# hguo/ftk

Hardware: AMD Instinct MI355X
Metric: space-time simplices/sec (higher is better)
Workload: dtype int64

## Files before the change

ftk_amd/__init__.py:

```python
import ctypes as C

import numpy as np

from . import _lib
from ._lib import (CP_DTYPE, FORMAT_BINARY, FORMAT_JSON, FORMAT_TEXT, SCOPE_BOTH, SCOPE_INTERVAL, SCOPE_ORDINAL, SOURCE_DERIVED, SOURCE_GIVEN, SOURCE_NONE,
                   TAG_EXACT64, TAG_REFERENCE, TAG_WORK_INDEX, FtkxError, Options, Stats)

__all__ = ["trace_curves", "pass2", "trace_and_post_process", "post_process", "post_process_curves", "TrajectorySet", "write_critical_points", "read_critical_points",
           "write_traced_critical_points", "read_traced_critical_points", "Context", "CriticalPointTracker2DRegular", "CriticalPointTracker3DRegular", "extract_cp2dt", "extract_cp3dt",
           "scaling_factor", "gaussian_kernel", "gaussian_kernel1d", "CP_DTYPE", "FtkxError"]


def _ptr(a):
    if a is None:
        return None, None, 0, False
    if isinstance(a, int):
        return a, None, 1, False
    if hasattr(a, "data_ptr"):
        if a.dtype.is_floating_point and a.element_size() not in (4, 8):
            raise TypeError("fields must be float64 or float32")
        a = a.contiguous()
        return a.data_ptr(), a, 1 if a.is_cuda else 0, bool(a.dtype.is_floating_point and a.element_size() == 4)
    if isinstance(a, np.ndarray) and a.dtype == np.float32:
        a = np.ascontiguousarray(a)
# ... 471 lines not shown

    def sweep_collect(self, copy=True):
        out, n = C.c_void_p(), C.c_size_t()
        self._ck(self._L.ftkx_sweep_collect(self._h, C.byref(out), C.byref(n)))
        return _lib.records_from(out.value, n.value, copy)

    def stats(self):
        s = Stats()
        self._ck(self._L.ftkx_get_stats(self._h, C.byref(s)))
        return {k: getattr(s, k) for k, _ in Stats._fields_}

    KERNELS = ("mask_kernel", "cull_kernel", "exact_kernel", "tile_kernel")

    def invalidate_masks(self):
        self._ck(self._L.ftkx_invalidate_masks(self._h))

    def set_profiling(self, on=True):
        self._ck(self._L.ftkx_set_profiling(self._h, int(on)))

    def debug_tile_repeat(self, repeat):
        self._ck(self._L.ftkx_debug_tile_repeat(self._h, int(repeat)))

    def upload_counts(self):
        a = C.c_ulonglong(0); b = C.c_ulonglong(0)
        self._ck(self._L.ftkx_debug_upload_counts(self._h, C.byref(a), C.byref(b)))
        return int(a.value), int(b.value)

    def kernel_times(self):
        ms = (C.c_double * 4)(); n = (C.c_ulonglong * 4)()
        self._ck(self._L.ftkx_get_kernel_times(self._h, ms, n))
# ... 571 lines not shown
```

ftk_amd/_lib.py:

```python
import ctypes as C
import os

import numpy as np

_HERE = os.path.dirname(os.path.abspath(__file__))
LIB_PATH = os.path.join(_HERE, "libftkx.so")

CP_DTYPE = np.dtype([("x", "<f8", (3,)), ("t", "<f8"), ("scalar", "<f8", (3,)), ("type", "<u4"), ("aux", "<u4"), ("tag", "<u8")])
assert CP_DTYPE.itemsize == 72

OK, E_INVALID, E_DEVICE, E_NOMEM, E_NOSLICE, E_UNSUPPORTED = 0, -1, -2, -3, -4, -5
SCOPE_ORDINAL, SCOPE_INTERVAL, SCOPE_BOTH = 1, 2, 3
TAG_WORK_INDEX, TAG_REFERENCE, TAG_EXACT64 = 0, 1, 2
FORMAT_BINARY, FORMAT_JSON, FORMAT_TEXT = 0, 1, 2
SOURCE_NONE, SOURCE_GIVEN, SOURCE_DERIVED = 0, 1, 2


class Options(C.Structure):
    _fields_ = [("jacobian_symmetric", C.c_int), ("robust", C.c_int), ("use_type_filter", C.c_int), ("type_filter", C.c_uint),
                ("compute_degrees", C.c_int), ("tag_mode", C.c_int), ("exact_only", C.c_int), ("derive_jacobian", C.c_int),
                ("coords_mode", C.c_int), ("coords_bounds", C.c_double * 6)]


class Stats(C.Structure):
# ... 44 lines not shown
    _fields_ = [("rank", C.c_int), ("nranks", C.c_int), ("t0", C.c_int), ("t1", C.c_int), ("lower", C.c_int), ("upper", C.c_int), ("bytes_sent", C.c_ulonglong),
                ("bytes_received", C.c_ulonglong), ("fallbacks", C.c_int), ("last_asked", C.c_longlong), ("last_served", C.c_longlong), ("last_path", C.c_int),
                ("last_status", C.c_ulonglong), ("open", C.c_int)]


class FtkxError(RuntimeError):
    def __init__(self, code, msg):
        super().__init__(f"ftkx error {code}: {msg}")
        self.code = code


EXPORTS = [
    "ftkx_create", "ftkx_destroy", "ftkx_last_error", "ftkx_set_stream", "ftkx_set_options", "ftkx_default_options", "ftkx_set_mesh",
    "ftkx_push_slice", "ftkx_push_scalar_slice", "ftkx_drop_slice", "ftkx_slice_resolution", "ftkx_slices_resolution", "ftkx_slices_prepare", "ftkx_sweep_announce", "ftkx_set_slice_resolution", "ftkx_export_masks_size", "ftkx_export_masks", "ftkx_push_masked_slice", "ftkx_packed_masks_bytes", "ftkx_export_masks_packed", "ftkx_push_masked_slice_packed", "ftkx_sweep_cull", "ftkx_get_sparse_cells", "ftkx_patch_doubles", "ftkx_gather_patches", "ftkx_scatter_patches", "ftkx_scaling_factor",
    "ftkx_sweep", "ftkx_sweep_series", "ftkx_sweep_series_submit", "ftkx_sweep_series_complete", "ftkx_sweep_series_abort", "ftkx_series_dist_cells", "ftkx_series_dist_begin", "ftkx_series_dist_cull", "ftkx_series_dist_serve", "ftkx_series_dist_finish", "ftkx_series_dist_status", "ftkx_series_last_path", "ftkx_series_split_decision", "ftkx_sweep_enqueue", "ftkx_sweep_enqueue_many", "ftkx_sweep_collect", "ftkx_sweep_cancel", "ftkx_get_stats", "ftkx_invalidate_masks", "ftkx_debug_stream_read", "ftkx_debug_tile_repeat", "ftkx_set_profiling", "ftkx_get_kernel_times", "ftkx_extract_cp2dt", "ftkx_extract_cp3dt", "ftkx_free",
    "ftkx_trace_curves", "ftkx_trace_curves_ctx", "ftkx_trace_curves_tags_ctx", "ftkx_trace_curves_device", "ftkx_trace_last_path", "ftkx_free_curves", "ftkx_post_process_curves", "ftkx_post_process_curves_device", "ftkx_pass2_device", "ftkx_post_process_last_path", "ftkx_free_trajectories", "ftkx_format_from_path", "ftkx_write_critical_points", "ftkx_read_critical_points", "ftkx_write_traced_critical_points", "ftkx_read_traced_critical_points", "ftkx_gradient2D", "ftkx_jacobian2D", "ftkx_gradient3D", "ftkx_jacobian3D", "ftkx_gaussian_kernel", "ftkx_conv2D", "ftkx_conv3D", "ftkx_set_spatial_smoothing", "ftkx_tracker_set_spatial_smoothing", "ftkx_debug_conv_relaunch", "ftkx_gaussian_kernel1d", "ftkx_temporal_combine", "ftkx_set_temporal_smoothing", "ftkx_temporal_push", "ftkx_temporal_flush", "ftkx_debug_temporal_relaunch", "ftkx_tracker_set_temporal_smoothing", "ftkx_tracker_snapshots_from_last_push", "ftkx_tracker_flush_temporal_smoothing", "ftkx_tracker_reset", "ftkx_version", "ftkx_device_count", "ftkx_pointer_device", "ftkx_context_device", "ftkx_last_mask_kernel", "ftkx_debug_mask_kernel_launches", "ftkx_debug_upload_counts", "ftkx_debug_mask_relaunch",
    "ftkx_push_scalar_slice_f32", "ftkx_push_slice_f32", "ftkx_temporal_push_f32", "ftkx_widen_f32", "ftkx_conv2D_f32", "ftkx_conv3D_f32", "ftkx_debug_widen_relaunch", "ftkx_debug_f32_counts", "ftkx_debug_array_counts",
    "ftkx_push_slice_planar", "ftkx_push_slice_planar_f32", "ftkx_temporal_push_planar", "ftkx_temporal_push_planar_f32", "ftkx_concat", "ftkx_concat_f32", "ftkx_debug_concat_relaunch", "ftkx_debug_planar_counts",
    "ftkx_tracker_push_vector_field_components", "ftkx_tracker_push_vector_field_components_f32",
    "ftkx_debug_series_order", "ftkx_debug_sort_records",
    "ftkx_set_perturbation", "ftkx_set_clamp", "ftkx_adjust", "ftkx_adjust_f32", "ftkx_debug_adjust_relaunch", "ftkx_debug_adjust_counts", "ftkx_tracker_set_perturbation", "ftkx_tracker_set_clamp",
    "ftkx_push_aux_slice", "ftkx_push_aux_slice_f32", "ftkx_sample_aux", "ftkx_debug_sample_relaunch", "ftkx_debug_sample_counts",
    "ftkx_tracker_set_scalar_components", "ftkx_tracker_push_snapshot_extra", "ftkx_tracker_get_curve_scalars",
    "ftkx_tracker_push_scalar_field_snapshot_f32", "ftkx_tracker_push_vector_field_snapshot_f32", "ftkx_tracker_push_field_data_snapshot_f32",
    "ftkx_tracker_post_process", "ftkx_tracker_get_curve_points", "ftkx_tracker_write", "ftkx_tracker_read_critical_points",
    "ftkx_tracker_create", "ftkx_tracker_create_multi", "ftkx_tracker_sync", "ftkx_tracker_destroy", "ftkx_tracker_last_error", "ftkx_tracker_set_domain", "ftkx_tracker_set_array_domain",
    "ftkx_tracker_set_sources", "ftkx_tracker_set_flags", "ftkx_tracker_set_stream", "ftkx_tracker_set_current_timestep", "ftkx_tracker_set_enable_streaming_trajectories", "ftkx_tracker_set_deferred_collection", "ftkx_tracker_set_trace_on_device", "ftkx_tracker_trace_last_path", "ftkx_tracker_set_post_process_on_device", "ftkx_tracker_post_process_last_path", "ftkx_tracker_set_communicator", "ftkx_tracker_set_slab_transport", "ftkx_tracker_set_slab_hub", "ftkx_online_tracer_create", "ftkx_online_tracer_destroy", "ftkx_online_tracer_grow", "ftkx_online_tracer_curves", "ftkx_tracker_set_coords_bounds", "ftkx_tracker_set_coords_rectilinear", "ftkx_tracker_set_coords_explicit", "ftkx_set_coords_rectilinear", "ftkx_set_coords_explicit", "ftkx_tracker_initialize",
    "ftkx_tracker_push_scalar_field_snapshot", "ftkx_tracker_push_vector_field_snapshot", "ftkx_tracker_push_field_data_snapshot",
    "ftkx_tracker_advance_timestep", "ftkx_tracker_update_timestep", "ftkx_tracker_num_critical_points",
    "ftkx_tracker_get_critical_points", "ftkx_tracker_get_scaling", "ftkx_tracker_get_stats",
    "ftkx_tracker_finalize", "ftkx_tracker_num_curves", "ftkx_tracker_get_curves",
# ... 28 lines not shown
    L.ftkx_push_scalar_slice.argtypes = [vp, C.c_int, dbl, C.c_int]
    L.ftkx_drop_slice.argtypes = [vp, C.c_int]
    L.ftkx_slice_resolution.argtypes = [vp, C.c_int, C.POINTER(C.c_double), C.POINTER(C.c_double)]
    L.ftkx_set_slice_resolution.argtypes = [vp, C.c_int, C.c_double, C.c_double]
    L.ftkx_scaling_factor.argtypes = [C.c_double, C.POINTER(C.c_int)]; L.ftkx_scaling_factor.restype = C.c_ulonglong
    L.ftkx_sweep.argtypes = [vp, C.c_int, C.c_int, C.c_ulonglong, C.POINTER(vp), C.POINTER(C.c_size_t)]
    L.ftkx_sweep_enqueue.argtypes = [vp, C.c_int, C.c_int, C.c_ulonglong]
    L.ftkx_sweep_collect.argtypes = [vp, C.POINTER(vp), C.POINTER(C.c_size_t)]
    L.ftkx_get_stats.argtypes = [vp, C.POINTER(Stats)]
    L.ftkx_set_profiling.argtypes = [vp, C.c_int]
    L.ftkx_invalidate_masks.argtypes = [vp]
    L.ftkx_debug_stream_read.argtypes = [vp, vp, C.c_size_t]
    L.ftkx_debug_tile_repeat.argtypes = [vp, C.c_int]
    L.ftkx_debug_upload_counts.argtypes = [vp, C.POINTER(C.c_ulonglong), C.POINTER(C.c_ulonglong)]
    L.ftkx_debug_mask_relaunch.argtypes = [vp, C.c_int, C.c_int, C.c_int, C.c_int, C.POINTER(C.c_double)]
    L.ftkx_series_split_decision.argtypes = [vp, C.POINTER(C.c_int), C.POINTER(C.c_double), C.POINTER(C.c_double)]
    L.ftkx_get_kernel_times.argtypes = [vp, C.POINTER(C.c_double), C.POINTER(C.c_ulonglong)]
    L.ftkx_extract_cp2dt.argtypes = [C.c_int, C.c_int] + [ll3] * 6 + [dbl] * 6 + [C.c_int, dbl, C.c_ulonglong, C.POINTER(Options), C.c_int, C.POINTER(vp), C.POINTER(C.c_size_t)]
    L.ftkx_extract_cp3dt.argtypes = [C.c_int, C.c_int] + [ll3] * 6 + [dbl] * 6 + [C.c_ulonglong, C.POINTER(Options), C.c_int, C.POINTER(vp), C.POINTER(C.c_size_t)]
    L.ftkx_free.argtypes = [vp]; L.ftkx_free.restype = None
    L.ftkx_trace_curves.argtypes = [C.c_int, ll3, ll3, vp, C.c_size_t, C.POINTER(Curves)]
    L.ftkx_trace_curves_ctx.argtypes = [vp, C.c_int, ll3, ll3, vp, C.c_size_t, C.POINTER(Curves)]
    L.ftkx_trace_curves_tags_ctx.argtypes = [vp, C.c_int, ll3, ll3, vp, C.c_size_t, C.POINTER(Curves)]
    L.ftkx_trace_curves_device.argtypes = [vp, C.c_int, ll3, ll3, vp, C.c_size_t, C.c_int, C.POINTER(Curves)]
    L.ftkx_trace_last_path.argtypes = [vp]
    L.ftkx_free_curves.argtypes = [C.POINTER(Curves)]; L.ftkx_free_curves.restype = None
    L.ftkx_post_process_curves.argtypes = [vp, C.c_size_t, C.POINTER(Curves), C.POINTER(Trajectories)]
    L.ftkx_post_process_curves_device.argtypes = [vp, vp, C.c_size_t, C.POINTER(Curves), C.POINTER(Trajectories)]
    L.ftkx_pass2_device.argtypes = [vp, C.c_int, ll3, ll3, vp, C.c_size_t, C.POINTER(Curves), C.POINTER(Trajectories)]
    L.ftkx_post_process_last_path.argtypes = [vp]
# ... 196 lines not shown
```

ftk_amd/csrc/mask_kernels.hip:

```cpp
#include <atomic>
#include "internal.hpp"
#include "mask_plan.hpp"
#include "sweep_device.hpp"
#include "series_device.hpp"

namespace ftkx {

__device__ inline void red_commit(u64 *red, double mn, double mx, unsigned slot)
{
  for (int o = 32; o > 0; o >>= 1) { mn = fmin(mn, __shfl_down(mn, o)); mx = fmax(mx, __shfl_down(mx, o)); }
  if ((threadIdx.x & 63) == 0) {
    atomicMin(&red[2 * (slot & 63u)], (u64)__double_as_longlong(mn));
    atomicMax(&red[2 * (slot & 63u) + 1], (u64)__double_as_longlong(mx));
  }
}

template <int ND>
__global__ __launch_bounds__(kThreads) void mask_kernel(const Mesh m, const MaskJob *__restrict__ jobs)
{
  const MaskJob job = jobs[blockIdx.y];
  const int P = m.mask_pitch, DH = m.ext_sz[1], DD = (ND == 3) ? m.ext_sz[2] : 1;
  const size_t n = (size_t)P * DH * DD;
  double red_mn = DBL_MAX, red_mx = 0.0;
  for (size_t idx = (size_t)blockIdx.x * kThreads + threadIdx.x; idx < n; idx += (size_t)gridDim.x * kThreads) {
    const int i = (int)(idx % P), j = (int)((idx / P) % DH), k = (int)(idx / ((size_t)P * DH));
    unsigned char mk = kNeutral;
    if (i < m.ext_sz[0]) {
      const int vx[3] = {i + m.ext_st[0], j + m.ext_st[1], k + m.ext_st[2]};
      bool in_dom = true;
      for (int d = 0; d < ND; d ++) in_dom = in_dom && vx[d] >= m.dom_lb[d] && vx[d] <= m.dom_ub[d];
      double v[ND];
      vector_at<ND>(m, job.S, job.V, i, j, k, v);
      unsigned bits = 0;
// ... 97 lines not shown
#define FTKX_GLOBAL __attribute__((address_space(1)))

__device__ inline double dpp_lower_or(double v, double edge)
{
  const long long b = __double_as_longlong(v), e = __double_as_longlong(edge);
  const int lo = __builtin_amdgcn_update_dpp((int)e, (int)b, 0x138 , 0xf, 0xf, false);
  const int hi = __builtin_amdgcn_update_dpp((int)(e >> 32), (int)(b >> 32), 0x138, 0xf, 0xf, false);
  return __longlong_as_double(((long long)hi << 32) | (unsigned)lo);
}
__device__ inline double dpp_upper_or(double v, double edge)
{
  const long long b = __double_as_longlong(v), e = __double_as_longlong(edge);
  const int lo = __builtin_amdgcn_update_dpp((int)e, (int)b, 0x130 , 0xf, 0xf, false);
  const int hi = __builtin_amdgcn_update_dpp((int)(e >> 32), (int)(b >> 32), 0x130, 0xf, 0xf, false);
  return __longlong_as_double(((long long)hi << 32) | (unsigned)lo);
}

__device__ inline void remap_block(int swizzle, unsigned &bx, unsigned &by, unsigned &bz)
{
  bx = blockIdx.x; by = blockIdx.y; bz = blockIdx.z;
  if (swizzle & 1) {
    const unsigned nb = gridDim.x * gridDim.y * gridDim.z;
    unsigned b = blockIdx.x + gridDim.x * (blockIdx.y + gridDim.y * blockIdx.z);
    const unsigned per = nb / 8, rem = nb % 8, xcd = b % 8, k = b / 8;
    b = xcd * per + (xcd < rem ? xcd : rem) + k;
    bx = b % gridDim.x; by = (b / gridDim.x) % gridDim.y; bz = b / (gridDim.x * gridDim.y);
  }
  if (swizzle & 8) {
    const unsigned YG = ((unsigned)swizzle >> 8) & 0xffu;
    const unsigned nb = gridDim.x * gridDim.y * gridDim.z, G = gridDim.x * YG;
// ... 80 lines not shown
  return __longlong_as_double(((long long)hi << 32) | (unsigned)lo);
}

__device__ inline unsigned word_summary(unsigned bits)
{
  unsigned q;
  asm("v_and_b32_sdwa %0, %1, %1 dst_sel:DWORD dst_unused:UNUSED_PAD src0_sel:BYTE_0 src1_sel:BYTE_1\n\t"
      "s_nop 1\n\t"
      "v_and_b32_dpp %0, %0, %0 quad_perm:[1,0,3,2] row_mask:0xf bank_mask:0xf\n\t"
      "s_nop 1\n\t"
      "v_and_b32_dpp %0, %0, %0 quad_perm:[2,3,0,1] row_mask:0xf bank_mask:0xf"
      : "=&v"(q) : "v"(bits));
  return q;
}

__device__ inline double max_abs2(double a, double b) { double r; asm("v_max_f64 %0, |%1|, |%2|" : "=v"(r) : "v"(a), "v"(b)); return r; }
__device__ inline double max_with_abs(double acc, double b) { asm("v_max_f64 %0, %0, |%1|" : "+v"(acc) : "v"(b)); return acc; }
__device__ inline double max_plain(double acc, double b) { asm("v_max_f64 %0, %0, %1" : "+v"(acc) : "v"(b)); return acc; }

template <int ND>
__device__ inline unsigned guard_and_reduce(unsigned a0, unsigned a1, double dx0, double dx1, double dy0, double dy1, double dz0, double dz1,
                                            bool rv, unsigned cmask, bool per_vertex_rule, double tbig, double h, double &acc0, double &acc1, double &red_mn)
{
  double m0 = max_abs2(dx0, dy0), m1 = max_abs2(dx1, dy1);
  if constexpr (ND == 3) { m0 = max_with_abs(m0, dz0); m1 = max_with_abs(m1, dz1); }
  unsigned bits = a0 | (a1 << 8);
  if (rv) {
    acc0 = max_plain(acc0, m0); acc1 = max_plain(acc1, m1);
    const unsigned u = bits | (bits >> 3);
    if (__builtin_amdgcn_ballot_w64((~u & cmask) != 0u)) {
      auto take = [&](double d) { const double a = fabs(h * d); red_mn = fmin(red_mn, a == 0.0 ? DBL_MAX : a); };
      if (cmask & 0x00ffu) { take(dx0); take(dy0); if (ND == 3) take(dz0); }
      if (cmask & 0xff00u) { take(dx1); take(dy1); if (ND == 3) take(dz1); }
// ... 958 lines not shown
  case MASK_ROWS2: hipLaunchKernelGGL(mask_rows2_kernel<8>, grid, block, 0, stream, m, d_jobs, p.groups, p.swizzle); break;
  case MASK_REDUCE:
    if (m.nd == 2) hipLaunchKernelGGL((mask_march4_kernel<2, true, 1, 8>), grid, block, 0, stream, m, d_jobs, p.zchunk, p.swizzle);
    else hipLaunchKernelGGL((mask_march4_kernel<3, true, 1, 4>), grid, block, 0, stream, m, d_jobs, p.zchunk, p.swizzle);
    break;
  case MASK_MARCH4: hipLaunchKernelGGL((mask_march4_kernel<2, false, 1, 8>), grid, block, 0, stream, m, d_jobs, p.zchunk, p.swizzle); break;
  case MASK_VEC2:
    if (m.nd == 2) hipLaunchKernelGGL(mask_vec2_kernel<2>, grid, block, 0, stream, m, d_jobs);
    else hipLaunchKernelGGL(mask_vec2_kernel<3>, grid, block, 0, stream, m, d_jobs);
    break;
  case MASK_VEC:
    if (m.nd == 2) hipLaunchKernelGGL(mask_vec_kernel<2>, grid, block, 0, stream, m, d_jobs);
    else hipLaunchKernelGGL(mask_vec_kernel<3>, grid, block, 0, stream, m, d_jobs);
    break;
  default:
    if (m.nd == 2) hipLaunchKernelGGL(mask_kernel<2>, grid, block, 0, stream, m, d_jobs);
    else hipLaunchKernelGGL(mask_kernel<3>, grid, block, 0, stream, m, d_jobs);
  }
}

void launch_masks(const Mesh &m, const MaskJob *d_jobs, int njobs, hipStream_t stream) { launch_masks_impl(m, d_jobs, njobs, false, stream); }
void launch_reduce_march(const Mesh &m, const MaskJob *d_jobs, int njobs, hipStream_t stream) { launch_masks_impl(m, d_jobs, njobs, true, stream); }

}
```

ftk_amd/csrc/mask_plan.hpp:

```cpp
#pragma once
#include <algorithm>
#include <cstdlib>
#include <cstring>
#include <vector>

namespace ftkx {

struct ZPlan {
  unsigned npieces;
  unsigned z0[47], len[47];
  unsigned sgroup;
};

#if defined(__HIPCC__)
#define FTKX_PLAN_HD __host__ __device__
#else
#define FTKX_PLAN_HD
#endif

struct ZWhere { unsigned job, piece; };
FTKX_PLAN_HD inline ZWhere zplan_decode(const ZPlan &plan, int njobs, unsigned bz)
{
  ZWhere w;
  if (njobs >= 0) { w.piece = bz / (unsigned)njobs; w.job = bz - w.piece * (unsigned)njobs; return w; }
  const unsigned nj = (unsigned)-njobs, t = bz / plan.npieces;
  if (plan.sgroup == 0) { w.piece = bz - t * plan.npieces; w.job = t; return w; }
  const unsigned ngroups = (nj + plan.sgroup - 1) / plan.sgroup, small = nj / ngroups, extra = nj - small * ngroups, head = extra * (small + 1);
  const unsigned size = t < head ? small + 1 : small;
  const unsigned first = t < head ? t / size * size : head + (t - head) / size * size;
  const unsigned r = bz - first * plan.npieces;
  w.piece = r / size; w.job = first + (r - w.piece * size);
  return w;
}

constexpr long kHookUnset = -0x7fffffffL;
struct MaskHooks {
  long swizzle = kHookUnset, yg = kHookUnset, zchunk = kHookUnset, lmin = kHookUnset, lcap = kHookUnset, order = kHookUnset, sgroup = kHookUnset, rows = kHookUnset, lean = kHookUnset;
  long u_rows = 0;
};
inline long hook_or(long v, long dflt) { return v == kHookUnset ? dflt : v; }

inline MaskHooks parse_mask_hooks(const char *plan, const char *u_rows)
{
  MaskHooks h;
  const struct { const char *name; long MaskHooks::*knob; } knobs[] = {{"swizzle", &MaskHooks::swizzle}, {"yg", &MaskHooks::yg}, {"zchunk", &MaskHooks::zchunk},
    {"lmin", &MaskHooks::lmin}, {"lcap", &MaskHooks::lcap}, {"order", &MaskHooks::order}, {"sgroup", &MaskHooks::sgroup}, {"rows", &MaskHooks::rows}, {"lean", &MaskHooks::lean}};
  for (const char *p = plan ? plan : ""; *p;) {
    while (*p == ',' || *p == ' ') p ++;
    for (const auto &k : knobs) {
      const size_t n = strlen(k.name);
      if (!strncmp(p, k.name, n) && p[n] == '=' && h.*k.knob == kHookUnset) h.*k.knob = atol(p + n + 1);
    }
    while (*p && *p != ',') p ++;
  }
  if (u_rows) h.u_rows = atoi(u_rows);
  return h;
}
inline MaskHooks read_mask_hooks() { return parse_mask_hooks(getenv("FTKX_MASK_PLAN"), getenv("FTKX_U_ROWS")); }

struct MaskShape { int nd, scalar_mode, ext_sz[3], mask_pitch; };

enum MaskFamily { MASK_MARCH6 = 0 , MASK_MARCH4 = 1 , MASK_ROWS2 = 2 ,
                  MASK_REDUCE = 3 , MASK_VEC2 = 4 ,
                  MASK_VEC = 5 , MASK_GENERIC = 6, MASK_FAMILIES = 7 };
constexpr unsigned kMaskThreads = 256;

struct MaskPlan {
  MaskFamily family;
  const char *name;
  bool march2;
  bool has_summary;
  int u_rows;
  unsigned grid[3], block, lds_bytes;
  int swizzle, zchunk, groups, njobs;
  ZPlan z;
};

inline MaskPlan plan_masks(const MaskShape &s, const MaskHooks &h, int njobs, bool reduce)
{
  MaskPlan p = MaskPlan();
  const int DW = s.ext_sz[0], DH = s.ext_sz[1], DD = s.nd == 3 ? s.ext_sz[2] : 1;
  const size_t nrows = (size_t)DH * (size_t)DD;
  p.march2 = s.scalar_mode && (DW % 2) == 0 && DW >= 2 && (size_t)DW * nrows * 8 < (1ull << 32);
  const bool vec_fast = !s.scalar_mode && DW >= 8 && (DW % 8) == 0;
  const bool vec_lean = vec_fast && DW >= 256 && hook_or(h.lean, 1) != 0 && (size_t)DW * nrows * 8 * (size_t)s.nd < (1ull << 31) && (size_t)s.mask_pitch * nrows < (1ull << 31);
  p.has_summary = h.u_rows >= 0 && (s.scalar_mode ? p.march2 && (DW % 8) == 0 : vec_fast);
  if (!p.has_summary || h.u_rows == 1) p.u_rows = 1;
  else if (!s.scalar_mode) p.u_rows = vec_lean ? 4 : 1;
  else if (s.nd == 3) p.u_rows = h.u_rows == 4 ? 4 : 16;
  else p.u_rows = 4;
// ... 81 lines not shown
  if (vec_fast) {
    const size_t groups = (size_t)(DW / 4) * nrows;
    size_t bx = (groups + kMaskThreads - 1) / kMaskThreads;
    if (bx > 2048) bx = 2048;
    while (bx > 256 && bx * kMaskThreads * 4 > groups) bx /= 2;
    if (p.u_rows == 4) {
      const size_t units = (size_t)((DW / 4 + 63) / 64) * ((DH + 3) / 4) * (size_t)DD;
      bx = (units + 7) / 8;
      if (bx > 2048) bx = 2048;
    }
    p.grid[0] = (unsigned)bx;
    p.family = p.u_rows == 4 ? MASK_VEC2 : MASK_VEC;
    p.name = p.u_rows == 4 ? (s.nd == 2 ? "ftkx::mask_vec2_kernel<2>" : "ftkx::mask_vec2_kernel<3>") : (s.nd == 2 ? "ftkx::mask_vec_kernel<2>" : "ftkx::mask_vec_kernel<3>");
    return p;
  }
  const size_t n = (size_t)s.mask_pitch * nrows;
  size_t bx = (n + kMaskThreads - 1) / kMaskThreads;
  if (bx > 4096) bx = 4096;
  p.grid[0] = (unsigned)bx;
  p.family = MASK_GENERIC; p.name = s.nd == 2 ? "ftkx::mask_kernel<2>" : "ftkx::mask_kernel<3>";
  return p;
}

}
```

ftk_amd/csrc/prepare.hip:

```cpp
#include "ctx.hpp"

using namespace ftkxh;

namespace ftkxh {

__global__ void init_red_kernel(u64 *red, size_t nslots, u64 *counters)
{
  const size_t i = (size_t)blockIdx.x * blockDim.x + threadIdx.x;
  if (i < nslots) { red[2 * i] = 0x7fefffffffffffffull; red[2 * i + 1] = 0ull; }
  if (counters && i < (size_t)ftkx::CNT_N) counters[i] = 0ull;
}

__global__ __launch_bounds__(256) void readback_kernel(const u64 *__restrict__ red, u64 *dst, unsigned k, unsigned *flag, unsigned seq)
{
  const unsigned wv = threadIdx.x >> 6, lane = threadIdx.x & 63;
  for (unsigned base = wv * 8; base < k; base += 32) {
    u64 mn[8], mx[8];
#pragma unroll
    for (int j = 0; j < 8; j ++) {
      const unsigned i = base + j < k ? base + j : k - 1;
      mn[j] = red[(size_t)i * 128 + 2 * lane]; mx[j] = red[(size_t)i * 128 + 2 * lane + 1];
    }
#pragma unroll
    for (int j = 0; j < 8; j ++) {
// ... 201 lines not shown
    hipStream_t q = st[r % nstreams];
    if (with_begin) launch_fetch_desc(c->h_desc.p, (char *)c->d_desc.p + 4096, 4096, q);
    ftkx::launch_masks(m, (const MaskJob *)c->d_desc.p, 1, q);
  }
  if (nstreams == 2) { HIP_TRY(c, hipEventRecord(eb, st[1])); HIP_TRY(c, hipStreamWaitEvent(st[0], eb, 0)); }
  HIP_TRY(c, hipEventRecord(e1, st[0]));
  HIP_TRY(c, hipEventSynchronize(e1));
  float ms = 0.f;
  HIP_TRY(c, hipEventElapsedTime(&ms, e0, e1));
  (void)hipEventDestroy(e0); (void)hipEventDestroy(e1); (void)hipEventDestroy(eb);
  if (st[1]) aux_stream_put(c, false, st[1]);
  *ms_per_launch = (double)ms / reps;
  return FTKX_OK;
}

int ftkx_sweep_announce(ftkx_ctx *c, const int *ts, const int *scopes, int n)
{
  if (!c || (n > 0 && (!ts || !scopes))) return fail(c, FTKX_E_INVALID, "null argument");
  c->announced.clear();
  for (int i = 0; i < n; i ++) {
    if (scopes[i] < FTKX_SCOPE_ORDINAL || scopes[i] > FTKX_SCOPE_BOTH) { c->announced.clear(); return fail(c, FTKX_E_INVALID, "ftkx_sweep_announce: bad scope %d", scopes[i]); }
    c->announced.push_back({ts[i], scopes[i]});
  }
  return FTKX_OK;
}

}
```

include/ftkx.h:

```cpp
#ifndef FTKX_H
#define FTKX_H

#include <stddef.h>

#ifdef __cplusplus
extern "C" {
#endif

typedef struct ftkx_cp_t {
  double x[3];
  double t;
  double scalar[3];
  unsigned int type;
  unsigned long long tag;
} ftkx_cp_t;

static inline unsigned int ftkx_cp_aux(const ftkx_cp_t *cp) { return ((const unsigned int *)cp)[15]; }
static inline int ftkx_cp_ordinal(const ftkx_cp_t *cp) { return (int)(ftkx_cp_aux(cp) & 1u); }
static inline int ftkx_cp_timestep(const ftkx_cp_t *cp) { return (int)(ftkx_cp_aux(cp) >> 1); }

typedef struct ftkx_ctx ftkx_ctx;

enum {
  FTKX_OK = 0,
// ... 215 lines not shown
int ftkx_debug_series_order(const ftkx_ctx *ctx, unsigned long long out[4]);
int ftkx_debug_sort_records(ftkx_ctx *ctx, const ftkx_cp_t *in, size_t n, int key_bits, ftkx_cp_t *out);

int ftkx_debug_stream_read(ftkx_ctx *ctx, const void *device_ptr, size_t bytes);

int ftkx_debug_tile_repeat(ftkx_ctx *ctx, int repeat);

const char *ftkx_last_mask_kernel(void);

int ftkx_debug_mask_kernel_launches(unsigned long long *launches, const char **names, int n);

int ftkx_debug_upload_counts(const ftkx_ctx *ctx, unsigned long long *staged, unsigned long long *direct);

int ftkx_debug_mask_relaunch(ftkx_ctx *ctx, int t, int reps, int nstreams, int with_begin, double *ms_per_launch);

const char *ftkx_version(void);
int ftkx_device_count(void);
int ftkx_pointer_device(const void *p);
int ftkx_context_device(const ftkx_ctx *ctx);

#ifdef __cplusplus
}
#endif
#endif
```

Measured before the change: 45990 billion.

## Replace generic byte mask kernel with wave-strided row-run tiled mask kernel

```diff
diff --git a/ftk_amd/__init__.py b/ftk_amd/__init__.py
--- a/ftk_amd/__init__.py
+++ b/ftk_amd/__init__.py
@@ -509,6 +509,10 @@
 
     def invalidate_masks(self):
         self._ck(self._L.ftkx_invalidate_masks(self._h))
+
+    def debug_mask_slices(self, ts, threshold, big, M_ptr, red_ptr):
+        ts = [int(t) for t in ts]
+        self._ck(self._L.ftkx_debug_mask_slices(self._h, (C.c_int * len(ts))(*ts), len(ts), float(threshold), float(big), M_ptr, red_ptr))
 
     def set_profiling(self, on=True):
         self._ck(self._L.ftkx_set_profiling(self._h, int(on)))
diff --git a/ftk_amd/_lib.py b/ftk_amd/_lib.py
--- a/ftk_amd/_lib.py
+++ b/ftk_amd/_lib.py
@@ -82,7 +82,7 @@
     "ftkx_create", "ftkx_destroy", "ftkx_last_error", "ftkx_set_stream", "ftkx_set_options", "ftkx_default_options", "ftkx_set_mesh",
     "ftkx_push_slice", "ftkx_push_scalar_slice", "ftkx_drop_slice", "ftkx_slice_resolution", "ftkx_slices_resolution", "ftkx_slices_prepare", "ftkx_sweep_announce", "ftkx_set_slice_resolution", "ftkx_export_masks_size", "ftkx_export_masks", "ftkx_push_masked_slice", "ftkx_packed_masks_bytes", "ftkx_export_masks_packed", "ftkx_push_masked_slice_packed", "ftkx_sweep_cull", "ftkx_get_sparse_cells", "ftkx_patch_doubles", "ftkx_gather_patches", "ftkx_scatter_patches", "ftkx_scaling_factor",
     "ftkx_sweep", "ftkx_sweep_series", "ftkx_sweep_series_submit", "ftkx_sweep_series_complete", "ftkx_sweep_series_abort", "ftkx_series_dist_cells", "ftkx_series_dist_begin", "ftkx_series_dist_cull", "ftkx_series_dist_serve", "ftkx_series_dist_finish", "ftkx_series_dist_status", "ftkx_series_last_path", "ftkx_series_split_decision", "ftkx_sweep_enqueue", "ftkx_sweep_enqueue_many", "ftkx_sweep_collect", "ftkx_sweep_cancel", "ftkx_get_stats", "ftkx_invalidate_masks", "ftkx_debug_stream_read", "ftkx_debug_tile_repeat", "ftkx_set_profiling", "ftkx_get_kernel_times", "ftkx_extract_cp2dt", "ftkx_extract_cp3dt", "ftkx_free",
-    "ftkx_trace_curves", "ftkx_trace_curves_ctx", "ftkx_trace_curves_tags_ctx", "ftkx_trace_curves_device", "ftkx_trace_last_path", "ftkx_free_curves", "ftkx_post_process_curves", "ftkx_post_process_curves_device", "ftkx_pass2_device", "ftkx_post_process_last_path", "ftkx_free_trajectories", "ftkx_format_from_path", "ftkx_write_critical_points", "ftkx_read_critical_points", "ftkx_write_traced_critical_points", "ftkx_read_traced_critical_points", "ftkx_gradient2D", "ftkx_jacobian2D", "ftkx_gradient3D", "ftkx_jacobian3D", "ftkx_gaussian_kernel", "ftkx_conv2D", "ftkx_conv3D", "ftkx_set_spatial_smoothing", "ftkx_tracker_set_spatial_smoothing", "ftkx_debug_conv_relaunch", "ftkx_gaussian_kernel1d", "ftkx_temporal_combine", "ftkx_set_temporal_smoothing", "ftkx_temporal_push", "ftkx_temporal_flush", "ftkx_debug_temporal_relaunch", "ftkx_tracker_set_temporal_smoothing", "ftkx_tracker_snapshots_from_last_push", "ftkx_tracker_flush_temporal_smoothing", "ftkx_tracker_reset", "ftkx_version", "ftkx_device_count", "ftkx_pointer_device", "ftkx_context_device", "ftkx_last_mask_kernel", "ftkx_debug_mask_kernel_launches", "ftkx_debug_upload_counts", "ftkx_debug_mask_relaunch",
+    "ftkx_trace_curves", "ftkx_trace_curves_ctx", "ftkx_trace_curves_tags_ctx", "ftkx_trace_curves_device", "ftkx_trace_last_path", "ftkx_free_curves", "ftkx_post_process_curves", "ftkx_post_process_curves_device", "ftkx_pass2_device", "ftkx_post_process_last_path", "ftkx_free_trajectories", "ftkx_format_from_path", "ftkx_write_critical_points", "ftkx_read_critical_points", "ftkx_write_traced_critical_points", "ftkx_read_traced_critical_points", "ftkx_gradient2D", "ftkx_jacobian2D", "ftkx_gradient3D", "ftkx_jacobian3D", "ftkx_gaussian_kernel", "ftkx_conv2D", "ftkx_conv3D", "ftkx_set_spatial_smoothing", "ftkx_tracker_set_spatial_smoothing", "ftkx_debug_conv_relaunch", "ftkx_gaussian_kernel1d", "ftkx_temporal_combine", "ftkx_set_temporal_smoothing", "ftkx_temporal_push", "ftkx_temporal_flush", "ftkx_debug_temporal_relaunch", "ftkx_tracker_set_temporal_smoothing", "ftkx_tracker_snapshots_from_last_push", "ftkx_tracker_flush_temporal_smoothing", "ftkx_tracker_reset", "ftkx_version", "ftkx_device_count", "ftkx_pointer_device", "ftkx_context_device", "ftkx_last_mask_kernel", "ftkx_debug_mask_kernel_launches", "ftkx_debug_upload_counts", "ftkx_debug_mask_relaunch", "ftkx_debug_mask_slices",
     "ftkx_push_scalar_slice_f32", "ftkx_push_slice_f32", "ftkx_temporal_push_f32", "ftkx_widen_f32", "ftkx_conv2D_f32", "ftkx_conv3D_f32", "ftkx_debug_widen_relaunch", "ftkx_debug_f32_counts", "ftkx_debug_array_counts",
     "ftkx_push_slice_planar", "ftkx_push_slice_planar_f32", "ftkx_temporal_push_planar", "ftkx_temporal_push_planar_f32", "ftkx_concat", "ftkx_concat_f32", "ftkx_debug_concat_relaunch", "ftkx_debug_planar_counts",
     "ftkx_tracker_push_vector_field_components", "ftkx_tracker_push_vector_field_components_f32",
@@ -141,6 +141,7 @@
     L.ftkx_debug_tile_repeat.argtypes = [vp, C.c_int]
     L.ftkx_debug_upload_counts.argtypes = [vp, C.POINTER(C.c_ulonglong), C.POINTER(C.c_ulonglong)]
     L.ftkx_debug_mask_relaunch.argtypes = [vp, C.c_int, C.c_int, C.c_int, C.c_int, C.POINTER(C.c_double)]
+    L.ftkx_debug_mask_slices.argtypes = [vp, C.POINTER(C.c_int), C.c_int, C.c_double, C.c_double, vp, vp]
     L.ftkx_series_split_decision.argtypes = [vp, C.POINTER(C.c_int), C.POINTER(C.c_double), C.POINTER(C.c_double)]
     L.ftkx_get_kernel_times.argtypes = [vp, C.POINTER(C.c_double), C.POINTER(C.c_ulonglong)]
     L.ftkx_extract_cp2dt.argtypes = [C.c_int, C.c_int] + [ll3] * 6 + [dbl] * 6 + [C.c_int, dbl, C.c_ulonglong, C.POINTER(Options), C.c_int, C.POINTER(vp), C.POINTER(C.c_size_t)]
diff --git a/ftk_amd/csrc/mask_generic_steps.hpp b/ftk_amd/csrc/mask_generic_steps.hpp
--- /dev/null
+++ b/ftk_amd/csrc/mask_generic_steps.hpp
@@ -0,0 +1,70 @@
+#pragma once
+#include <cstddef>
+
+#if defined(__HIPCC__)
+#define GEN_HD __host__ __device__ inline
+#else
+#define GEN_HD inline
+#endif
+
+namespace ftkx {
+
+constexpr int kGenCols = 64;
+
+template <int ND, bool SCALAR> struct GenTile {
+  static constexpr int RY = SCALAR ? (ND == 3 ? 4 : 8) : 4;
+  static constexpr int ZC = (SCALAR && ND == 3) ? 32 : 1;
+};
+
+struct GenWalk {
+  int DW, DH, DD, P;
+  int RY, ZC;
+  unsigned nseg, nruns, nzc, nunits;
+};
+
+struct GenUnit { unsigned seg, run, zc; };
+
+GEN_HD GenWalk gen_walk(int DW, int DH, int DD, int P, int RY, int ZC)
+{
+  GenWalk w;
+  w.DW = DW; w.DH = DH; w.DD = DD; w.P = P; w.RY = RY; w.ZC = ZC;
+  w.nseg = ((unsigned)P + (unsigned)kGenCols - 1u) / (unsigned)kGenCols;
+  w.nruns = ((unsigned)DH + (unsigned)RY - 1u) / (unsigned)RY;
+  w.nzc = ((unsigned)DD + (unsigned)ZC - 1u) / (unsigned)ZC;
+  w.nunits = w.nseg * w.nruns * w.nzc;
+  return w;
+}
+
+GEN_HD GenUnit gen_decode(const GenWalk &w, unsigned u)
+{
+  GenUnit at;
+  const unsigned t = u / w.nseg;
+  at.seg = u - t * w.nseg;
+  at.zc = t / w.nruns;
+  at.run = t - at.zc * w.nruns;
+  return at;
+}
+
+GEN_HD void gen_advance(const GenWalk &w, GenUnit &at, const GenUnit &d)
+{
+  at.seg += d.seg; at.run += d.run; at.zc += d.zc;
+  if (at.seg >= w.nseg) { at.seg -= w.nseg; at.run ++; }
+  if (at.run >= w.nruns) { at.run -= w.nruns; at.zc ++; }
+}
+
+GEN_HD int gen_clamp(int i, int lo, int hi) { return i < lo ? lo : (i > hi ? hi : i); }
+
+GEN_HD size_t gen_row(const GenWalk &w, int j, int k)
+{
+  return ((size_t)gen_clamp(k, 0, w.DD - 1) * (size_t)w.DH + (size_t)gen_clamp(j, 0, w.DH - 1)) * (size_t)w.DW;
+}
+GEN_HD size_t gen_mask_row(const GenWalk &w, int j, int k) { return ((size_t)k * (size_t)w.DH + (size_t)j) * (size_t)w.P; }
+
+GEN_HD unsigned gen_col(const GenWalk &w, unsigned seg, unsigned lane) { return (unsigned)gen_clamp((int)(seg * kGenCols + lane), 0, w.DW - 1); }
+GEN_HD unsigned gen_edge_col(const GenWalk &w, unsigned seg, unsigned lane)
+{
+  const int x0 = (int)(seg * kGenCols);
+  return (unsigned)gen_clamp(lane < 32u ? x0 - 1 : x0 + kGenCols, 0, w.DW - 1);
+}
+
+}
diff --git a/ftk_amd/csrc/mask_kernels.hip b/ftk_amd/csrc/mask_kernels.hip
--- a/ftk_amd/csrc/mask_kernels.hip
+++ b/ftk_amd/csrc/mask_kernels.hip
@@ -1,6 +1,7 @@
 #include <atomic>
 #include "internal.hpp"
 #include "mask_plan.hpp"
+#include "mask_generic_steps.hpp"
 #include "sweep_device.hpp"
 #include "series_device.hpp"
 
@@ -16,7 +17,7 @@
 }
 
 template <int ND>
-__global__ __launch_bounds__(kThreads) void mask_kernel(const Mesh m, const MaskJob *__restrict__ jobs)
+__global__ __launch_bounds__(kThreads) void mask_bytes_kernel(const Mesh m, const MaskJob *__restrict__ jobs)
 {
   const MaskJob job = jobs[blockIdx.y];
   const int P = m.mask_pitch, DH = m.ext_sz[1], DD = (ND == 3) ? m.ext_sz[2] : 1;
@@ -144,6 +145,214 @@
   const int lo = __builtin_amdgcn_update_dpp((int)e, (int)b, 0x130 , 0xf, 0xf, false);
   const int hi = __builtin_amdgcn_update_dpp((int)(e >> 32), (int)(b >> 32), 0x130, 0xf, 0xf, false);
   return __longlong_as_double(((long long)hi << 32) | (unsigned)lo);
+}
+
+__device__ inline double max_abs2(double a, double b) { double r; asm("v_max_f64 %0, |%1|, |%2|" : "=v"(r) : "v"(a), "v"(b)); return r; }
+__device__ inline double max_with_abs(double acc, double b) { asm("v_max_f64 %0, %0, |%1|" : "+v"(acc) : "v"(b)); return acc; }
+__device__ inline double max_plain(double acc, double b) { asm("v_max_f64 %0, %0, %1" : "+v"(acc) : "v"(b)); return acc; }
+
+__device__ inline unsigned quad_word(unsigned b)
+{
+  const unsigned h = b | ((unsigned)__builtin_amdgcn_update_dpp(0, (int)b, 0xf5 , 0xf, 0xf, false) << 8);
+  return h | ((unsigned)__builtin_amdgcn_update_dpp(0, (int)h, 0xee , 0xf, 0xf, false) << 16);
+}
+
+template <int ND>
+__device__ inline unsigned gen_classify(const double (&v)[ND], bool keep, double thr, double big, double &red_mn, double &red_mx)
+{
+  unsigned bits = 0;
+  bool finite = true, isbig = false, cand = false;
+#pragma unroll
+  for (int c = 0; c < ND; c ++) {
+    const double a = fabs(v[c]);
+    finite = finite && a < HUGE_VAL;
+    if (v[c] >= thr) bits |= 1u << c;
+    if (v[c] <= -thr) bits |= 8u << c;
+    isbig = isbig || a >= big;
+    red_mx = fmax(red_mx, a);
+    cand = cand || (a < thr && a != 0.0);
+  }
+  if (__builtin_amdgcn_ballot_w64(cand)) {
+#pragma unroll
+    for (int c = 0; c < ND; c ++) { const double a = fabs(v[c]); red_mn = fmin(red_mn, (a == 0.0 || !(a < thr)) ? DBL_MAX : a); }
+  }
+  return (keep && finite) ? (isbig ? 0u : bits) : (unsigned)kNeutral;
+}
+
+struct GenLoop {
+  GenWalk w; GenUnit at, d; unsigned u, W, lane;
+  bool any;
+  __device__ GenLoop(const Mesh &m, int nd, int RY, int ZC)
+  {
+    lane = threadIdx.x & 63u;
+    W = gridDim.x * (unsigned)(kThreads / 64);
+    w = gen_walk(m.ext_sz[0], m.ext_sz[1], nd == 3 ? m.ext_sz[2] : 1, m.mask_pitch, RY, ZC);
+    u = blockIdx.x * (unsigned)(kThreads / 64) + (unsigned)__builtin_amdgcn_readfirstlane((int)(threadIdx.x >> 6));
+    any = u < w.nunits;
+    at = GenUnit{0u, 0u, 0u}; d = at;
+    if (any) { at = gen_decode(w, u); d = gen_decode(w, W); }
+  }
+  __device__ bool more()
+  {
+    u = (unsigned)__builtin_amdgcn_readfirstlane((int)u); at.seg = (unsigned)__builtin_amdgcn_readfirstlane((int)at.seg);
+    at.run = (unsigned)__builtin_amdgcn_readfirstlane((int)at.run); at.zc = (unsigned)__builtin_amdgcn_readfirstlane((int)at.zc);
+    return u < w.nunits;
+  }
+  __device__ void next() { u += W; gen_advance(w, at, d); }
+};
+
+__device__ inline bool gen_in_dom(const Mesh &m, int a, int i) { return i + m.ext_st[a] >= m.dom_lb[a] && i + m.ext_st[a] <= m.dom_ub[a]; }
+
+__device__ inline bool gen_scalar3(const Mesh &m, const MaskJob &job, int tune, double &red_mn, double &red_mx)
+{
+  typedef GenTile<3, true> T;
+  constexpr int RY = T::RY;
+  GenLoop L(m, 3, RY, tune > 0 ? tune : T::ZC);
+  const GenWalk &w = L.w;
+  const FTKX_GLOBAL double *S = (const FTKX_GLOBAL double *)job.S;
+  FTKX_GLOBAL unsigned char *M = (FTKX_GLOBAL unsigned char *)job.M;
+  const double thr = job.threshold, big = job.big, tp = 2.0 * thr, tn = -tp;
+  for (; L.more(); L.next()) {
+    const unsigned c = gen_col(w, L.at.seg, L.lane), e = gen_edge_col(w, L.at.seg, L.lane);
+    const int x = (int)(L.at.seg * kGenCols + L.lane), j0 = (int)L.at.run * RY, z0 = (int)L.at.zc * w.ZC, z1 = z0 + w.ZC < w.DD ? z0 + w.ZC : w.DD;
+    const bool x_int = x >= 1 && x < w.DW - 1, x_dom = x < w.DW && gen_in_dom(m, 0, x);
+    const bool store = (L.lane & 3u) == 0u && x < w.P;
+    const size_t ro0 = gen_row(w, j0 - 1, 0);
+    unsigned ro[RY + 2];
+#pragma unroll
+    for (int r = 0; r < RY + 2; r ++) ro[r] = (unsigned)(gen_row(w, j0 - 1 + r, 0) - ro0);
+    auto load = [&](double (&B)[RY + 2], double (&E)[RY], int k, bool edges) {
+      const FTKX_GLOBAL double *pl = S + (gen_row(w, 0, k) + ro0);
+#pragma unroll
+      for (int r = 0; r < RY + 2; r ++) B[r] = (pl + ro[r])[c];
+      if (edges) {
+#pragma unroll
+        for (int r = 0; r < RY; r ++) E[r] = (pl + ro[r + 1])[e];
+      }
+    };
+    auto rows = [&](const double (&A)[RY + 2], const double (&B)[RY + 2], const double (&C)[RY + 2], const double (&E)[RY], int k) {
+      int jb = j0;
+      asm volatile("" : "+s"(jb));
+      const bool k_int = k >= 1 && k < w.DD - 1, k_dom = gen_in_dom(m, 2, k);
+      FTKX_GLOBAL unsigned char *Mk = M + gen_mask_row(w, 0, k);
+#pragma unroll
+      for (int r = 0; r < RY; r ++) {
+        const int j = jb + r;
+        if (j < w.DH) {
+          const double xm = dpp_lower_or(B[r + 1], E[r]), xp = dpp_upper_or(B[r + 1], E[r]);
+          const double dx = xp - xm, dy = B[r + 2] - B[r], dz = C[r + 1] - A[r + 1];
+          const bool in = x_int && k_int && j >= 1 && j < w.DH - 1;
+          unsigned bits = (dx >= tp ? 1u : 0u) | (dy >= tp ? 2u : 0u) | (dz >= tp ? 4u : 0u) | (dx <= tn ? 8u : 0u) | (dy <= tn ? 16u : 0u) | (dz <= tn ? 32u : 0u);
+          const bool fin = fabs(dx) < HUGE_VAL && fabs(dy) < HUGE_VAL && fabs(dz) < HUGE_VAL;
+          double am = 0.5 * max_with_abs(max_abs2(dx, dy), dz);
+          bits = in ? bits : 0u; am = in ? am : 0.0;
+          red_mx = max_plain(red_mx, am);
+          if (__builtin_amdgcn_ballot_w64(in && ((bits | (bits >> 3)) & 7u) != 7u)) {
+            const double d[3] = {dx, dy, dz};
+#pragma unroll
+            for (int q = 0; q < 3; q ++) { const double a = in ? fabs(0.5 * d[q]) : 0.0; red_mn = fmin(red_mn, (a == 0.0 || !(a < thr)) ? DBL_MAX : a); }
+          }
+          const bool keep = x_dom && k_dom && gen_in_dom(m, 1, j) && (fin || !in);
+          const unsigned word = quad_word(keep ? (am >= big ? 0u : bits) : (unsigned)kNeutral);
+          if (store) *reinterpret_cast<FTKX_GLOBAL unsigned *>(Mk + gen_mask_row(w, j, 0) + (unsigned)x) = word;
+        }
+      }
+    };
+    double PA[RY + 2], PB[RY + 2], PC[RY + 2], PD[RY + 2], EA[RY], EB[RY], EC[RY], ED[RY];
+    load(PA, EA, z0 - 1, false); load(PB, EB, z0, true); load(PC, EC, z0 + 1, true);
+    for (int k = z0; k < z1; k += 4) {
+      load(PD, ED, k + 2, true); if (k < z1) rows(PA, PB, PC, EB, k);
+      load(PA, EA, k + 3, true); if (k + 1 < z1) rows(PB, PC, PD, EC, k + 1);
+      load(PB, EB, k + 4, true); if (k + 2 < z1) rows(PC, PD, PA, ED, k + 2);
+      load(PC, EC, k + 5, true); if (k + 3 < z1) rows(PD, PA, PB, EA, k + 3);
+    }
+  }
+  return L.any;
+}
+
+__device__ inline bool gen_scalar2(const Mesh &m, const MaskJob &job, double &red_mn, double &red_mx)
+{
+  constexpr int RY = GenTile<2, true>::RY;
+  GenLoop L(m, 2, RY, 1);
+  const GenWalk &w = L.w;
+  const FTKX_GLOBAL double *S = (const FTKX_GLOBAL double *)job.S;
+  FTKX_GLOBAL unsigned char *M = (FTKX_GLOBAL unsigned char *)job.M;
+  const double thr = job.threshold, big = job.big, fx = (double)(w.DW - 1), fy = (double)(w.DH - 1);
+  for (; L.more(); L.next()) {
+    const unsigned c = gen_col(w, L.at.seg, L.lane), e = gen_edge_col(w, L.at.seg, L.lane);
+    const int x = (int)(L.at.seg * kGenCols + L.lane), j0 = (int)L.at.run * RY;
+    const bool live = x < w.DW, x_dom = live && gen_in_dom(m, 0, x);
+    const bool store = (L.lane & 3u) == 0u && x < w.P;
+    double B[RY + 2], E[RY];
+#pragma unroll
+    for (int r = 0; r < RY + 2; r ++) B[r] = (S + gen_row(w, j0 - 1 + r, 0))[c];
+#pragma unroll
+    for (int r = 0; r < RY; r ++) E[r] = (S + gen_row(w, j0 + r, 0))[e];
+#pragma unroll
+    for (int r = 0; r < RY; r ++) {
+      const int j = j0 + r;
+      if (j < w.DH) {
+        const double xm = dpp_lower_or(B[r + 1], E[r]), xp = dpp_upper_or(B[r + 1], E[r]);
+        const double g0 = (xp - xm) * fx, g1 = (B[r + 2] - B[r]) * fy;
+        const double v[2] = {live ? g0 : 0.0, live ? g1 : 0.0};
+        const unsigned word = quad_word(gen_classify<2>(v, x_dom && gen_in_dom(m, 1, j), thr, big, red_mn, red_mx));
+        if (store) *reinterpret_cast<FTKX_GLOBAL unsigned *>(M + gen_mask_row(w, j, 0) + (unsigned)x) = word;
+      }
+    }
+  }
+  return L.any;
+}
+
+template <int ND>
+__device__ inline bool gen_vector(const Mesh &m, const MaskJob &job, double &red_mn, double &red_mx)
+{
+  constexpr int RY = GenTile<ND, false>::RY;
+  GenLoop L(m, ND, RY, 1);
+  const GenWalk &w = L.w;
+  const FTKX_GLOBAL double *V = (const FTKX_GLOBAL double *)job.V;
+  FTKX_GLOBAL unsigned char *M = (FTKX_GLOBAL unsigned char *)job.M;
+  const double thr = job.threshold, big = job.big;
+  const bool wide = ND == 2 && ((size_t)job.V & 15u) == 0;
+  for (; L.more(); L.next()) {
+    const unsigned c = gen_col(w, L.at.seg, L.lane) * (unsigned)ND;
+    const int x = (int)(L.at.seg * kGenCols + L.lane), j0 = (int)L.at.run * RY, k = (int)L.at.zc;
+    const bool live = x < w.DW, x_dom = live && gen_in_dom(m, 0, x) && (ND == 2 || gen_in_dom(m, 2, k));
+    const bool store = (L.lane & 3u) == 0u && x < w.P;
+    double D[RY][ND];
+#pragma unroll
+    for (int r = 0; r < RY; r ++) {
+      const FTKX_GLOBAL double *row = V + gen_row(w, j0 + r, k) * (size_t)ND;
+      if (wide) { const v2d t = *reinterpret_cast<const FTKX_GLOBAL v2d *>(row + c); D[r][0] = t.x; D[r][ND - 1] = t.y; }
+      else {
+#pragma unroll
+        for (int q = 0; q < ND; q ++) D[r][q] = row[c + (unsigned)q];
+      }
+    }
+#pragma unroll
+    for (int r = 0; r < RY; r ++) {
+      const int j = j0 + r;
+      if (j < w.DH) {
+        double v[ND];
+#pragma unroll
+        for (int q = 0; q < ND; q ++) v[q] = live ? D[r][q] : 0.0;
+        const unsigned word = quad_word(gen_classify<ND>(v, x_dom && gen_in_dom(m, 1, j), thr, big, red_mn, red_mx));
+        if (store) *reinterpret_cast<FTKX_GLOBAL unsigned *>(M + gen_mask_row(w, j, k) + (unsigned)x) = word;
+      }
+    }
+  }
+  return L.any;
+}
+
+template <int ND>
+__global__ __launch_bounds__(kThreads) void mask_kernel(const Mesh m, const MaskJob *__restrict__ jobs, int tune)
+{
+  const MaskJob job = jobs[blockIdx.y];
+  double red_mn = DBL_MAX, red_mx = 0.0;
+  bool any;
+  if (!m.scalar_mode) any = gen_vector<ND>(m, job, red_mn, red_mx);
+  else if constexpr (ND == 3) any = gen_scalar3(m, job, tune, red_mn, red_mx);
+  else any = gen_scalar2(m, job, red_mn, red_mx);
+  if (job.red && any) red_commit(job.red, red_mn, red_mx, blockIdx.x * 5u + (threadIdx.x >> 6));
 }
 
 __device__ inline void remap_block(int swizzle, unsigned &bx, unsigned &by, unsigned &bz)
@@ -254,9 +463,6 @@
   return q;
 }
 
-__device__ inline double max_abs2(double a, double b) { double r; asm("v_max_f64 %0, |%1|, |%2|" : "=v"(r) : "v"(a), "v"(b)); return r; }
-__device__ inline double max_with_abs(double acc, double b) { asm("v_max_f64 %0, %0, |%1|" : "+v"(acc) : "v"(b)); return acc; }
-__device__ inline double max_plain(double acc, double b) { asm("v_max_f64 %0, %0, %1" : "+v"(acc) : "v"(b)); return acc; }
 
 template <int ND>
 __device__ inline unsigned guard_and_reduce(unsigned a0, unsigned a1, double dx0, double dx1, double dy0, double dy1, double dz0, double dz1,
@@ -1245,8 +1451,13 @@
     else hipLaunchKernelGGL(mask_vec_kernel<3>, grid, block, 0, stream, m, d_jobs);
     break;
   default:
-    if (m.nd == 2) hipLaunchKernelGGL(mask_kernel<2>, grid, block, 0, stream, m, d_jobs);
-    else hipLaunchKernelGGL(mask_kernel<3>, grid, block, 0, stream, m, d_jobs);
+    if (p.bytes_body) {
+      g_last_mask_kernel = m.nd == 2 ? "ftkx::mask_bytes_kernel<2>" : "ftkx::mask_bytes_kernel<3>";
+      if (m.nd == 2) hipLaunchKernelGGL(mask_bytes_kernel<2>, grid, block, 0, stream, m, d_jobs);
+      else hipLaunchKernelGGL(mask_bytes_kernel<3>, grid, block, 0, stream, m, d_jobs);
+    }
+    else if (m.nd == 2) hipLaunchKernelGGL(mask_kernel<2>, grid, block, 0, stream, m, d_jobs, p.tune);
+    else hipLaunchKernelGGL(mask_kernel<3>, grid, block, 0, stream, m, d_jobs, p.tune);
   }
 }
 
diff --git a/ftk_amd/csrc/mask_plan.hpp b/ftk_amd/csrc/mask_plan.hpp
--- a/ftk_amd/csrc/mask_plan.hpp
+++ b/ftk_amd/csrc/mask_plan.hpp
@@ -35,7 +35,7 @@
 
 constexpr long kHookUnset = -0x7fffffffL;
 struct MaskHooks {
-  long swizzle = kHookUnset, yg = kHookUnset, zchunk = kHookUnset, lmin = kHookUnset, lcap = kHookUnset, order = kHookUnset, sgroup = kHookUnset, rows = kHookUnset, lean = kHookUnset;
+  long swizzle = kHookUnset, yg = kHookUnset, zchunk = kHookUnset, lmin = kHookUnset, lcap = kHookUnset, order = kHookUnset, sgroup = kHookUnset, rows = kHookUnset, lean = kHookUnset, generic = kHookUnset, gunit = kHookUnset;
   long u_rows = 0;
 };
 inline long hook_or(long v, long dflt) { return v == kHookUnset ? dflt : v; }
@@ -44,7 +44,7 @@
 {
   MaskHooks h;
   const struct { const char *name; long MaskHooks::*knob; } knobs[] = {{"swizzle", &MaskHooks::swizzle}, {"yg", &MaskHooks::yg}, {"zchunk", &MaskHooks::zchunk},
-    {"lmin", &MaskHooks::lmin}, {"lcap", &MaskHooks::lcap}, {"order", &MaskHooks::order}, {"sgroup", &MaskHooks::sgroup}, {"rows", &MaskHooks::rows}, {"lean", &MaskHooks::lean}};
+    {"lmin", &MaskHooks::lmin}, {"lcap", &MaskHooks::lcap}, {"order", &MaskHooks::order}, {"sgroup", &MaskHooks::sgroup}, {"rows", &MaskHooks::rows}, {"lean", &MaskHooks::lean}, {"generic", &MaskHooks::generic}, {"gunit", &MaskHooks::gunit}};
   for (const char *p = plan ? plan : ""; *p;) {
     while (*p == ',' || *p == ' ') p ++;
     for (const auto &k : knobs) {
@@ -74,6 +74,8 @@
   unsigned grid[3], block, lds_bytes;
   int swizzle, zchunk, groups, njobs;
   ZPlan z;
+  int tune;
+  bool bytes_body;
 };
 
 inline MaskPlan plan_masks(const MaskShape &s, const MaskHooks &h, int njobs, bool reduce)
@@ -185,6 +187,8 @@
     p.name = p.u_rows == 4 ? (s.nd == 2 ? "ftkx::mask_vec2_kernel<2>" : "ftkx::mask_vec2_kernel<3>") : (s.nd == 2 ? "ftkx::mask_vec_kernel<2>" : "ftkx::mask_vec_kernel<3>");
     return p;
   }
+  p.bytes_body = hook_or(h.generic, 1) == 0;
+  { const long g = hook_or(h.gunit, 0); p.tune = (int)(g < 0 ? 0 : g > 4096 ? 4096 : g); }
   const size_t n = (size_t)s.mask_pitch * nrows;
   size_t bx = (n + kMaskThreads - 1) / kMaskThreads;
   if (bx > 4096) bx = 4096;
diff --git a/ftk_amd/csrc/prepare.hip b/ftk_amd/csrc/prepare.hip
--- a/ftk_amd/csrc/prepare.hip
+++ b/ftk_amd/csrc/prepare.hip
@@ -239,6 +239,30 @@
   return FTKX_OK;
 }
 
+int ftkx_debug_mask_slices(ftkx_ctx *c, const int *ts, int n, double threshold, double big, void *M_dst, unsigned long long *red_dst)
+{
+  if (!c || !ts || n < 1 || !M_dst || !red_dst || !(threshold > 0.0)) return fail(c, FTKX_E_INVALID, "ftkx_debug_mask_slices: bad argument");
+  if (!c->pending.empty() || c->sr_open) return fail(c, FTKX_E_INVALID, "ftkx_debug_mask_slices: sweeps pending or passes open");
+  Mesh m; fill_mesh(c, m);
+  if (ftkx::masks_have_summary(m)) return fail(c, FTKX_E_UNSUPPORTED, "ftkx_debug_mask_slices: this mesh has summarised masks");
+  HIP_TRY(c, hipSetDevice(c->device));
+  int rc;
+  if ((rc = ensure_desc(c, (size_t)n * sizeof(MaskJob)))) return rc;
+  const size_t mbytes = (size_t)m.mask_pitch * (size_t)m.ext_sz[1] * (size_t)(m.nd == 3 ? m.ext_sz[2] : 1);
+  MaskJob *jobs = (MaskJob *)c->h_desc.p;
+  for (int i = 0; i < n; i ++) {
+    auto it = c->slices.find(ts[i]);
+    if (it == c->slices.end() || it->second.sparse) return fail(c, FTKX_E_NOSLICE, "ftkx_debug_mask_slices: timestep %d not resident", ts[i]);
+    jobs[i] = with_lean_thresholds(MaskJob{it->second.S.as<double>(), it->second.V.as<double>(), (unsigned char *)M_dst + (size_t)i * mbytes, nullptr, (u64 *)red_dst + (size_t)i * 128, threshold, big}, m);
+  }
+  launch_init_red((u64 *)red_dst, (size_t)n * 64, nullptr, c->stream);
+  HIP_TRY(c, hipMemcpyAsync(c->d_desc.p, c->h_desc.p, (size_t)n * sizeof(MaskJob), hipMemcpyHostToDevice, c->stream));
+  ftkx::launch_masks(m, (const MaskJob *)c->d_desc.p, n, c->stream);
+  HIP_TRY(c, hipGetLastError());
+  HIP_TRY(c, hipStreamSynchronize(c->stream));
+  return FTKX_OK;
+}
+
 int ftkx_sweep_announce(ftkx_ctx *c, const int *ts, const int *scopes, int n)
 {
   if (!c || (n > 0 && (!ts || !scopes))) return fail(c, FTKX_E_INVALID, "null argument");
diff --git a/include/ftkx.h b/include/ftkx.h
--- a/include/ftkx.h
+++ b/include/ftkx.h
@@ -253,6 +253,8 @@
 
 int ftkx_debug_mask_relaunch(ftkx_ctx *ctx, int t, int reps, int nstreams, int with_begin, double *ms_per_launch);
 
+int ftkx_debug_mask_slices(ftkx_ctx *ctx, const int *ts, int n, double threshold, double big, void *M_dst, unsigned long long *red_dst);
+
 const char *ftkx_version(void);
 int ftkx_device_count(void);
 int ftkx_pointer_device(const void *p);
```

New measurement: 45920 billion. Within noise of the previous version (-0.1%).
